# gchq/annchor

Measured on AMD Instinct MI355X. Metric: knn_graph_builds_per_s (1 / Annchor.fit() wall-clock; BASELINE: k-NN graph build time + recall@k), higher is better.
Workload: dtype int32 bit-vectors (Levenshtein) + f64 (bounds/regression/selection); 1 GPU; load_strings Levenshtein N=1600 n_anchors=15 k=25 p_work=0.12 niters=2; parallelism=one GPU

## Files before the change

### annchor_amd/_native.py

```python
import ctypes
import os

import numpy as np

_HERE = os.path.dirname(os.path.abspath(__file__))
LIB_PATH = os.environ.get("ANNCHOR_HIP_LIB", os.path.join(_HERE, "libannchor_hip.so"))

F_D, F_A, F_SID, F_IJS, F_I_PTR, F_I_IDX, F_FEATURES, F_NCM, F_RA, F_LABELS, F_THRESH, F_PROB, F_CAND, F_NEXT, F_DAD = range(1, 16)
_FIELD_DTYPE = {
    F_D: np.float64, F_A: np.int64, F_SID: np.uint64, F_IJS: np.int64, F_I_PTR: np.int64, F_I_IDX: np.int64,
    F_FEATURES: np.float64, F_NCM: np.uint8, F_RA: np.float64, F_LABELS: np.int64, F_THRESH: np.float64,
    F_PROB: np.float64, F_CAND: np.int64, F_NEXT: np.int64, F_DAD: np.float64,
}

METRIC_LEVENSHTEIN, METRIC_EUCLIDEAN_F32, METRIC_EUCLIDEAN_F64, METRIC_WASSERSTEIN = 1, 2, 3, 4
METRIC_COSINE_F32, METRIC_COSINE_F64 = 5, 6
METRIC_DTW_F32, METRIC_DTW_F64 = 7, 8
METRIC_FRECHET_F32, METRIC_FRECHET_F64 = 9, 10

_vp, _i32, _i64, _dbl = ctypes.c_void_p, ctypes.c_int32, ctypes.c_int64, ctypes.c_double
_SIGNATURES = {
    "annchor_create": (ctypes.c_int, [ctypes.c_int, ctypes.POINTER(_vp)]),
    "annchor_destroy": (None, [_vp]),
    "annchor_release_parked": (ctypes.c_int, []),
    "annchor_parked_bytes": (ctypes.c_int, [ctypes.c_int, ctypes.POINTER(_i64)]),
    "annchor_last_error": (ctypes.c_char_p, [_vp]),
    "annchor_create_error": (ctypes.c_char_p, []),
    "annchor_device_name": (ctypes.c_int, [_vp, ctypes.c_char_p, ctypes.c_int]),
    "annchor_device_pci_bus_id": (ctypes.c_int, [ctypes.c_int, ctypes.c_char_p, ctypes.c_int]),
    "annchor_device_mem_info": (ctypes.c_int, [ctypes.c_int, ctypes.POINTER(_i64), ctypes.POINTER(_i64)]),
    "annchor_synchronize": (ctypes.c_int, [_vp]),
    "annchor_lev_persist_state": (ctypes.c_int, [ctypes.c_int]),
    "annchor_last_kernel_ms": (ctypes.c_int, [_vp, ctypes.POINTER(ctypes.c_float)]),
    "annchor_set_strings": (ctypes.c_int, [_vp, _vp, _vp, _vp, _i64, _i32]),
    "annchor_set_strings_u16": (ctypes.c_int, [_vp, _vp, _vp, _vp, _i64, _i32]),
    "annchor_set_points_f32": (ctypes.c_int, [_vp, _vp, _i64, _i32]),
    "annchor_set_points_f64": (ctypes.c_int, [_vp, _vp, _i64, _i32]),
    "annchor_set_points_cosine_f32": (ctypes.c_int, [_vp, _vp, _i64, _i32]),
    "annchor_set_points_cosine_f64": (ctypes.c_int, [_vp, _vp, _i64, _i32]),
    "annchor_set_series_f32": (ctypes.c_int, [_vp, _vp, _vp, _vp, _i64, _i32]),
    "annchor_set_series_f64": (ctypes.c_int, [_vp, _vp, _vp, _vp, _i64, _i32]),
    "annchor_set_curves_f32": (ctypes.c_int, [_vp, _vp, _vp, _vp, _i64, _i32]),
    "annchor_set_curves_f64": (ctypes.c_int, [_vp, _vp, _vp, _vp, _i64, _i32]),
    "annchor_set_histograms": (ctypes.c_int, [_vp, _vp, _i64, _i32, _vp]),
    "annchor_set_histograms_wide": (ctypes.c_int, [_vp, _vp, _i64, _i32, _vp]),
    "annchor_set_opaque": (ctypes.c_int, [_vp, _i64]),
    "annchor_metric_pairs": (ctypes.c_int, [_vp, _vp, _i64, _vp]),
# ... 351 lines not shown
        except Exception:
            pass

    def _chk(self, rc):
        if rc != 0:
            raise NativeError("libannchor_hip error %d: %s" % (rc, self.lib.annchor_last_error(self.h).decode()))

    def device_name(self):
        buf = ctypes.create_string_buffer(256)
        self._chk(self.lib.annchor_device_name(self.h, buf, 256))
        return buf.value.decode()

    def synchronize(self):
        self._chk(self.lib.annchor_synchronize(self.h))

    def last_kernel_ms(self):
        ms = ctypes.c_float()
        self._chk(self.lib.annchor_last_kernel_ms(self.h, ctypes.byref(ms)))
        return ms.value

    def set_strings(self, codes, offs, lens, alphabet):
        offs, lens = _c(offs, np.int64), _c(lens, np.int32)
        if np.asarray(codes).dtype == np.uint16:
            codes = _c(codes, np.uint16)
            self._chk(self.lib.annchor_set_strings_u16(self.h, _ptr(codes), _ptr(offs), _ptr(lens), len(lens), int(alphabet)))
        else:
            codes = _c(codes, np.uint8)
            self._chk(self.lib.annchor_set_strings(self.h, _ptr(codes), _ptr(offs), _ptr(lens), len(lens), int(alphabet)))
        self.nx, self.metric = len(lens), METRIC_LEVENSHTEIN

# ... 677 lines not shown
```

### annchor_amd/csrc/common.h

```cpp
#pragma once
#include <hip/hip_runtime.h>

#include <cstdint>
#include <cstdio>
#include <cstring>
#include <string>
#include <vector>
#include <chrono>

#include "../../include/annchor_hip.h"

#define ANN_WAVE 64

struct DevBuf {
    void *p = nullptr;
    size_t cap = 0;
    bool in_arena = false;
    template <typename T> T *as() const { return reinterpret_cast<T *>(p); }
};

struct ProfEntry {
    const char *name;
    double ms = 0;
    int64_t launches = 0;
// ... 15 lines not shown
    size_t arena_size = 0, arena_off = 0;

    int metric = ANNCHOR_METRIC_NONE;
    int64_t nx = 0;
    DevBuf sym, soff, slen;
    int alphabet = 0, maxlen = 0;
    bool sym_wide = false;
    int lev_gl0 = 0;
    double lev_frac0 = 0.0;
    DevBuf lev_order;
    int lev_nshort = 0;
    DevBuf lev_ap;
    DevBuf lev_ap_min;
    uint32_t lev_ap_epoch = 0;
    uint32_t lev_ap_probe_epoch = 0;
    DevBuf lev_cursors;
    int lev_cursor_epoch = 0;
    DevBuf lev_perm;
    DevBuf pts;
    int dtw_window = -1;
    int curve_dim = 0;
    int dim = 0;
    DevBuf hist, cost, supp;
    DevBuf hs_bin, hs_val, hs_cnt;
    int nbins = 0, max_support = 0;
    double cost_max = 0.0;
    int emd_epoch = 0;
    bool cost_is_metric = false;
    bool hist_integral = false;
    bool hist_fits_i16 = false;
// ... 121 lines not shown
        int _r = (expr);             \
        if (_r != ANNCHOR_OK) return _r; \
    } while (0)

#define ANN_REQUIRE(c, cond, code, ...)    \
    do {                                   \
        if (!(cond)) {                     \
            ann_set_err((c), __VA_ARGS__); \
            return (code);                 \
        }                                  \
    } while (0)

int ann_reserve(annchor_ctx *c, DevBuf &b, size_t bytes);
int ann_arena_init(annchor_ctx *c, int64_t nx);
int ann_prewarm_state(annchor_ctx *c);
void ann_lev_ap_probe(annchor_ctx *c);
size_t ann_sel2_table_bytes();
size_t ann_tie_hist_bytes();
size_t ann_sel_state_bytes();
int ann_h2d(annchor_ctx *c, void *dst, const void *src, size_t bytes);
hipError_t ann_sync(annchor_ctx *c, const char *where);
int ann_dev_alloc(annchor_ctx *c, void **p, size_t want, size_t *got);
void ann_dev_free(annchor_ctx *c, void *p, size_t bytes);
struct Sel2Epilogue;
int ann_kth_async(annchor_ctx *c, const double *vals, const uint8_t *flag, int64_t n, const int64_t *ks, int nk,
                  const unsigned long long **d_prefix, const int **d_unfinished, const Sel2Epilogue *epi = nullptr);
void ann_kth_async_done(annchor_ctx *c);
int ann_d2h(annchor_ctx *c, void *dst, const void *src, size_t bytes);
int ann_d2h_then(annchor_ctx *c, void *dst, const void *src, size_t bytes, int (*then)(annchor_ctx *));
int ann_d2h2(annchor_ctx *c, void *dst1, const void *src1, size_t bytes1, void *dst2, const void *src2, size_t bytes2);
// ... 169 lines not shown
```

### annchor_amd/csrc/ctx.hip

```cpp
#include <cstdarg>
#include <cmath>
#include <cstdlib>

#include "common.h"
#include <algorithm>
#include <chrono>
#include <mutex>

static std::string g_create_err;
void ann_stream_release(annchor_ctx *c);
void ann_enemies_release(annchor_ctx *c);
void ann_comm_release(annchor_ctx *c);
hipError_t ann_comm_guarded_sync(annchor_ctx *c, hipStream_t stream, const char *where);

const char *ann_set_err(annchor_ctx *c, const char *fmt, ...)
{
    char buf[1024];
    va_list ap;
    va_start(ap, fmt);
    vsnprintf(buf, sizeof buf, fmt, ap);
    va_end(ap);
    if (c && c->comm_aborted && c->err.rfind("collective timed out", 0) == 0) return c->err.c_str();
    if (c) c->err = buf; else g_create_err = buf;
    return c ? c->err.c_str() : g_create_err.c_str();
// ... 608 lines not shown
    }
    ANN_TRY(ann_arena_init(c, nx));
    ANN_TRY(ann_prewarm_state(c));
    ANN_TRY(ann_reserve(c, c->sym, pool.size() * sizeof(uint16_t)));
    ANN_TRY(ann_reserve(c, c->soff, sizeof(int32_t) * (size_t)nx));
    ANN_TRY(ann_reserve(c, c->slen, sizeof(int32_t) * (size_t)nx));
    ANN_TRY(ann_h2d(c, c->sym.p, pool.data(), pool.size() * sizeof(uint16_t)));
    ANN_TRY(ann_h2d(c, c->soff.p, o.data(), sizeof(int32_t) * (size_t)nx));
    ANN_TRY(ann_h2d(c, c->slen.p, lens, sizeof(int32_t) * (size_t)nx));
    c->metric = ANNCHOR_METRIC_LEVENSHTEIN;
    c->nx = nx;
    c->alphabet = alphabet;
    c->maxlen = maxlen;
    c->sym_wide = true;
    c->lev_gl0 = 0; c->lev_frac0 = 0.0; c->lev_nshort = 0;
    reset_pipeline(c);
    return ANNCHOR_OK;
}

extern "C" int annchor_set_strings(annchor_ctx *c, const uint8_t *symbols, const int64_t *offs,
                                   const int32_t *lens, int64_t nx, int32_t alphabet)
{
    if (!c || !symbols || !offs || !lens) return ANNCHOR_EINVAL;
    ANN_REQUIRE(c, nx > 1 && nx < (1ll << 31), ANNCHOR_ELIMIT, "nx=%lld out of range", (long long)nx);
    ANN_REQUIRE(c, alphabet >= 1 && alphabet <= 256, ANNCHOR_ELIMIT, "alphabet=%d not in 1..256", alphabet);
    ANN_CHECK_HIP(c, hipSetDevice(c->device));
    std::vector<int32_t> o((size_t)nx);
    size_t total = 0;
    int maxlen = 0;
    for (int64_t s = 0; s < nx; ++s) {
// ... 22 lines not shown
    c->metric = ANNCHOR_METRIC_LEVENSHTEIN;
    c->nx = nx;
    c->alphabet = alphabet;
    c->maxlen = maxlen;
    c->sym_wide = false;
    {
        std::vector<int32_t> ord((size_t)nx);
        int64_t ns = 0;
        for (int64_t s = 0; s < nx; ++s) ns += lens[s] <= 512;
        int64_t a = 0, b = ns;
        for (int64_t s = 0; s < nx; ++s) ord[(size_t)(lens[s] <= 512 ? a++ : b++)] = (int32_t)s;
        ANN_TRY(ann_reserve(c, c->lev_order, sizeof(int32_t) * (size_t)nx));
        ANN_TRY(ann_h2d(c, c->lev_order.p, ord.data(), sizeof(int32_t) * (size_t)nx));
        c->lev_nshort = (int)ns;
    }
    {
        const int W = (maxlen + 31) / 32 > 0 ? (maxlen + 31) / 32 : 1;
        c->lev_gl0 = 0;
        c->lev_frac0 = 0.0;
        if (W <= 32) {
            const int gl0 = 64 / (64 / W + 1);
            if (gl0 >= 1) {
                int64_t cnt = 0;
                for (int64_t s = 0; s < nx; ++s) cnt += (lens[s] + 31) / 32 <= gl0;
                c->lev_gl0 = gl0;
                c->lev_frac0 = (double)cnt / (double)nx;
            }
        }
    }
    reset_pipeline(c);
// ... 295 lines not shown
```

### annchor_amd/csrc/lev.hip

```cpp
#include <cstdlib>

#include "common.h"
#include <atomic>
#include <type_traits>

#define LEV_THREADS 256
#define LEV_WAVES (LEV_THREADS / ANN_WAVE)

__device__ __forceinline__ uint32_t dpp_wave_shr1(uint32_t v)
{
    return (uint32_t)__builtin_amdgcn_update_dpp((int)v, (int)v, 0x138 , 0xf, 0xf, false);
}

struct LevArgs {
    const uint8_t *sym;
    const int32_t *soff;
    const int32_t *slen;
    const int2 *ij;
    const int32_t *idx;
    const int32_t *anchor;
    int64_t n;
    double *out;
    double *RA;
    uint8_t *ncm;
// ... 899 lines not shown
    }
}


struct LevArgsAP {
    const uint8_t *sym;
    const int32_t *soff;
    const int32_t *slen;
    const int32_t *order;
    double *Dt;
    int32_t *A;
    int32_t *rank;
    unsigned long long *slots;
    uint32_t *abort_epoch;
    uint16_t *rescue_min;
    long long timeout_ticks;
    long long *dbg;
    uint32_t epoch;
    int n_short, nx, na, first, ntasks, slot_stride;
    int alphabet, pm_bytes, fb_stride, buf_stride, pad, wave_bytes;
};

template <bool RESCUE> __global__ __launch_bounds__(RESCUE ? 512 : ANN_WAVE) void k_lev_ap(LevArgsAP a)
{
    extern __shared__ __attribute__((aligned(16))) unsigned char smem_all[];
    __shared__ uint32_t s_best;
    __shared__ int32_t s_A[64];
    {
        const uint32_t ab = __hip_atomic_load(a.abort_epoch, __ATOMIC_RELAXED, __HIP_MEMORY_SCOPE_AGENT);
        if (RESCUE ? ab != a.epoch : ab == a.epoch) return;
    }
    const int lane = threadIdx.x & 63, wv = threadIdx.x >> 6, nwv = blockDim.x >> 6;
    unsigned char *smem = smem_all + (size_t)wv * a.wave_bytes;
    const int A = a.alphabet, nx = a.nx;
    unsigned char *pm_col = smem + (size_t)(lane >> 5) * A * LEVF_ROW + (size_t)(lane & 31) * 4;
// ... 6 lines not shown
    uint32_t rm0 = 0xffffu, rm1 = 0xffffu;
    int rk0 = -1, rk1 = -1;
    int si = a.first;
    for (int r = 0; r < a.na; ++r) {
        if (RESCUE) {
            if (threadIdx.x == 0) { s_best = 0; s_A[r] = si; }
            __syncthreads();
        }
#ifdef LEV_AP_PROFILE
#define AP_STAMP(i) do { if (!RESCUE && lane == 0) a.dbg[((size_t)blockIdx.x * 64 + r) * 8 + (i)] = (long long)__builtin_readcyclecounter(); } while (0)
#else
#define AP_STAMP(i) do { } while (0)
#endif
        AP_STAMP(0);
        if ((RESCUE ? threadIdx.x : blockIdx.x + lane) == 0) a.A[r] = si;
        const int la = a.slen[si];
        const uint8_t *asrc = a.sym + a.soff[si];
        uint32_t mykey = 0;
        for (int vb = RESCUE ? wv : (int)blockIdx.x; vb < a.ntasks; vb += RESCUE ? nwv : a.ntasks) {
            if (RESCUE || r == 0) {
                const bool packed = vb < ws;
                const int GL = packed ? 16 : 32;
                const int slot = lane / GL;
                w = lane - slot * GL; pair = slot >> 1; half = slot & 1; LP = packed ? 32 : 64;
                hp_or = w == 0 ? 0x80000000u : 0u;
                hn_and = w == 0 ? 0u : 0xffffffffu;
                asm volatile("" : "+v"(hp_or), "+v"(hn_and));
                tq0 = tq1 = -1;
                if (packed) {
                    tq0 = a.order[2 * vb];
                    if (2 * vb + 1 < a.n_short) tq1 = a.order[2 * vb + 1];
                } else {
                    tq0 = a.order[a.n_short + (vb - ws)];
                }
                for (int e = lane * 16; e < 3 * a.buf_stride; e += 64 * 16) *reinterpret_cast<uint4 *>(bufs + e) = make_uint4(0, 0, 0, 0);
                int ln0 = 0, ln1 = 0;
                {
                    ln0 = a.slen[tq0];
                    const uint8_t *src = a.sym + a.soff[tq0];
                    for (int ch = lane; ch < ((ln0 + 15) >> 4); ch += 64)
                        reinterpret_cast<uint4 *>(bufs + a.pad)[ch] = reinterpret_cast<const uint4 *>(src)[ch];
                }
                if (tq1 >= 0) {
                    ln1 = a.slen[tq1];
                    const uint8_t *src = a.sym + a.soff[tq1];
                    for (int ch = lane; ch < ((ln1 + 15) >> 4); ch += 64)
                        reinterpret_cast<uint4 *>(bufs + a.buf_stride + a.pad)[ch] = reinterpret_cast<const uint4 *>(src)[ch];
                }
                wave_lds_fence();
                have = pair == 0 || (packed && pair == 1 && tq1 >= 0);
                mytq = !have ? -1 : (pair == 0 ? tq0 : tq1);
                m = !have ? 0 : (pair == 0 ? ln0 : ln1);
                Wp = (m + 31) >> 5;
                const uint8_t *pat = bufs + pair * a.buf_stride + a.pad;
                for (int c = 0; c < A; ++c) *reinterpret_cast<uint32_t *>(pm_col + (size_t)c * LEVF_ROW) = 0u;
                if (have && w < Wp) {
                    const int valid = min(32, m - w * 32);
                    uint32_t sy[32];
                    if (half == 0) {
                        const uint4 *p16 = reinterpret_cast<const uint4 *>(pat + w * 32);
                        const uint4 q0 = p16[0], q1 = p16[1];
                        const uint32_t wd[8] = {q0.x, q0.y, q0.z, q0.w, q1.x, q1.y, q1.z, q1.w};
#pragma unroll
                        for (int k = 0; k < 32; ++k) sy[k] = (wd[k >> 2] >> ((k & 3) * 8)) & 0xffu;
                    } else {
#pragma unroll
                        for (int k = 0; k < 32; ++k) sy[k] = pat[max(m - 1 - (w * 32 + k), 0)];
                    }
#pragma unroll
                    for (int k = 0; k < 32; ++k)
                        if (k < valid) atomicOr(reinterpret_cast<uint32_t *>(pm_col + (size_t)sy[k] * LEVF_ROW), 1u << k);
                }
                rows = !have ? 0u : (w < Wp - 1 ? 0xffffffffu : (w == Wp - 1 ? (0xffffffffu >> (31 - ((m - 1) & 31))) : 0u));
            }
            for (int ch = lane; ch < ((la + 15) >> 4); ch += 64)
                reinterpret_cast<uint4 *>(bufs + 2 * a.buf_stride + a.pad)[ch] = reinterpret_cast<const uint4 *>(asrc)[ch];
            wave_lds_fence();
            AP_STAMP(1);
            const uint8_t *txt = bufs + 2 * a.buf_stride + a.pad;
            const int n = have ? la : 0;
            const int h = (n + 1) >> 1;
            const uint32_t un = (have && m > 0) ? (uint32_t)(half ? n - h : h) : 0u;
            int max_steps = (have && m > 0) ? h + Wp - 1 : 0;
            int k_lo = (have && m > 0) ? Wp - 1 : 0, k_hi = (have && m > 0) ? n - h : 0x7fffffff;
#pragma unroll
            for (int off = 32; off > 0; off >>= 1) {
                max_steps = max(max_steps, __shfl_xor(max_steps, off));
                k_lo = max(k_lo, __shfl_xor(k_lo, off));
                k_hi = min(k_hi, __shfl_xor(k_hi, off));
            }
            max_steps = __builtin_amdgcn_readfirstlane(max_steps);
// ... 51 lines not shown
            for (; k < k_hi; ++k) column1(k, std::false_type());
            for (; k < max_steps; ++k) column1(k, std::true_type());
            AP_STAMP(3);

            const int part = __popc(vp & rows) - __popc(vn & rows);
            int incl = part;
#pragma unroll
            for (int off = 1; off < 32; off <<= 1) {
                const int o = __shfl_up(incl, off, 32);
                if (w >= off) incl += o;
            }
            int val = (int)un + incl - part;
            if (m == 0) val = half ? n - h : h;
            int16_t *fbp = FB + (size_t)pair * 2 * a.fb_stride;
            int16_t *fb = fbp + (size_t)half * a.fb_stride;
            if (have && w == 0) fb[0] = (int16_t)val;
#pragma unroll
            for (int b = 0; b < 32; ++b) {
                val += (int)((vp >> b) & 1u) - (int)((vn >> b) & 1u);
                if ((rows >> b) & 1u) fb[w * 32 + b + 1] = (int16_t)val;
            }
            wave_lds_fence();
            int best = 0x7fffffff;
            const int lp = lane & (LP - 1);
            if (have)
                for (int i = lp; i <= m; i += LP) best = min(best, (int)fbp[i] + (int)fbp[a.fb_stride + m - i]);
#pragma unroll
            for (int off = 32; off > 0; off >>= 1)
                if (off < LP) best = min(best, __shfl_xor(best, off));
            if (have && lp == 0) a.Dt[(size_t)r * nx + mytq] = (double)best;
            wave_lds_fence();
            AP_STAMP(4);
            if (RESCUE) {
                if (have && lp == 0) {
                    uint32_t v = (uint32_t)best;
                    if (r > 1) v = min(v, (uint32_t)a.rescue_min[mytq]);
                    a.rescue_min[mytq] = (uint16_t)v;
                    atomicMax(&s_best, (v << 16) | (uint32_t)(0xffff - mytq));
                }
            } else {
                const uint32_t d0 = (uint32_t)__shfl(best, 0), d1 = (uint32_t)__shfl(best, 32);
                rm0 = r <= 1 ? d0 : min(rm0, d0);
                rm1 = r <= 1 ? d1 : min(rm1, d1);
                mykey = (rm0 << 16) | (uint32_t)(0xffff - tq0);
                if (tq1 >= 0) mykey = max(mykey, (rm1 << 16) | (uint32_t)(0xffff - tq1));
                if (si == tq0) rk0 = r;
                if (si == tq1) rk1 = r;
            }
        }
        if (r + 1 == a.na) break;
        if (RESCUE) {
            __syncthreads();
            si = 0xffff - (int)(s_best & 0xffffu);
            __syncthreads();
        } else {
            const uint32_t tag = a.epoch * 64u + (uint32_t)r;
            unsigned long long *sl = a.slots + (size_t)(r & 1) * a.slot_stride;
            unsigned long long *pl = sl + 2 * a.slot_stride;
            const int ngroups = (a.ntasks + 63) >> 6;
            if (lane == 0)
                __hip_atomic_store(sl + blockIdx.x, ((unsigned long long)tag << 32) | mykey, __ATOMIC_RELAXED, __HIP_MEMORY_SCOPE_AGENT);
            const long long t0 = wall_clock64();
            AP_STAMP(5);
            uint32_t mx;
            bool collected = (int)blockIdx.x >= ngroups;
            int polls = 0;
            for (;;) {
                if (!collected) {
                    const unsigned long long v = __hip_atomic_load(sl + min((int)blockIdx.x * 64 + lane, a.ntasks - 1), __ATOMIC_RELAXED,
                                                                   __HIP_MEMORY_SCOPE_AGENT);
                    if (__all((uint32_t)(v >> 32) == tag)) {
                        uint32_t gm = (uint32_t)v;
#pragma unroll
                        for (int off = 32; off > 0; off >>= 1) gm = max(gm, (uint32_t)__shfl_xor((int)gm, off));
                        if (lane == 0)
                            __hip_atomic_store(pl + blockIdx.x, ((unsigned long long)tag << 32) | gm, __ATOMIC_RELAXED, __HIP_MEMORY_SCOPE_AGENT);
// ... 19 lines not shown
            AP_STAMP(6);
        }
    }
    if (RESCUE) {
        __syncthreads();
        for (int j = threadIdx.x; j < nx; j += blockDim.x) a.rank[j] = -1;
        __syncthreads();
        if (threadIdx.x == 0)
            for (int r = 0; r < a.na; ++r) a.rank[s_A[r]] = r;
    } else {
        if (lane == 0) {
            a.rank[tq0] = rk0;
            if (tq1 >= 0) a.rank[tq1] = rk1;
        }
    }
}

static int launch_p2(annchor_ctx *c, const PairSource &src, double *d_out, double *d_RA, uint8_t *d_ncm)
{
    LevArgsP2 a;
    a.sym = c->sym.as<uint8_t>(); a.soff = c->soff.as<int32_t>(); a.slen = c->slen.as<int32_t>();
    a.ij = src.ij; a.idx = src.idx; a.n = src.n; a.out = d_out; a.RA = d_RA; a.ncm = d_ncm;
    a.alphabet = c->alphabet;
    a.pm_bytes = 2 * a.alphabet * LEVF_ROW;
    a.fb_stride = (c->maxlen + 2 + 7) & ~7;
    a.pad = ((c->maxlen / 2 + 48) + 15) & ~15;
    a.buf_stride = 2 * a.pad + ((c->maxlen + 15) & ~15) + 16;
    const size_t lds = (size_t)a.pm_bytes + 4 * (size_t)a.buf_stride + 4 * sizeof(int16_t) * a.fb_stride;
    ANN_REQUIRE(c, lds <= 160 * 1024, ANNCHOR_ELIMIT, "alphabet %d x length %d needs %zu B of LDS (> 160 KiB)", c->alphabet,
                c->maxlen, lds);
// ... 72 lines not shown
    if (set == 1) { g_lev_ap_off.store(0); g_lev_ap_strikes.store(0); }
    return g_lev_ap_off.load() ? 0 : 1;
}

int ann_lev_anchor_rounds(annchor_ctx *c, int32_t na, int32_t first, bool *done)
{
    *done = false;
    {
        const char *e = getenv("ANNCHOR_LEV_PERSIST");
        if (e && atoi(e) == 0) return ANNCHOR_OK;
        if (g_lev_ap_off.load()) return ANNCHOR_OK;
        const char *e_a = getenv("ANNCHOR_LEV_ANCHOR"), *e_r = getenv("ANNCHOR_LEV_R");
        if ((e_a && atoi(e_a) != 2) || e_r) return ANNCHOR_OK;
    }
    if (c->metric != ANNCHOR_METRIC_LEVENSHTEIN || c->sym_wide || !c->lev_order.p) return ANNCHOR_OK;
    if ((c->maxlen + 31) / 32 > 32 || c->nx > 8192 || na < 1 || na > 64) return ANNCHOR_OK;
    LevArgsAP a;
    a.ntasks = (c->lev_nshort + 1) / 2 + (int)(c->nx - c->lev_nshort);
    if (a.ntasks > 1024) return ANNCHOR_OK;
    a.alphabet = c->alphabet;
    a.pm_bytes = 2 * a.alphabet * LEVF_ROW;
    a.fb_stride = (c->maxlen + 2 + 7) & ~7;
    a.pad = ((c->maxlen / 2 + 48) + 15) & ~15;
    a.buf_stride = 2 * a.pad + ((c->maxlen + 15) & ~15) + 16;
    a.wave_bytes = (int)(((size_t)a.pm_bytes + 3 * (size_t)a.buf_stride + 4 * sizeof(int16_t) * a.fb_stride + 15) & ~(size_t)15);
    size_t lds = (size_t)a.wave_bytes;
    if (lds > 160 * 1024) return ANNCHOR_OK;
    if (a.ntasks <= c->prop.multiProcessorCount * 4 && lds < (size_t)40 * 1024) lds = (size_t)40 * 1024;
    if (lds > 64 * 1024)
        ANN_CHECK_HIP(c, hipFuncSetAttribute((const void *)k_lev_ap<false>, hipFuncAttributeMaxDynamicSharedMemorySize, (int)lds));
    int per_cu = 0;
    ANN_CHECK_HIP(c, hipOccupancyMaxActiveBlocksPerMultiprocessor(&per_cu, k_lev_ap<false>, ANN_WAVE, lds));
    if ((int64_t)per_cu * c->prop.multiProcessorCount < a.ntasks) return ANNCHOR_OK;
    int rwaves = (int)std::min<size_t>(8, (160 * 1024 - 1024) / (size_t)a.wave_bytes);
// ... 4 lines not shown
    a.slot_stride = 1024;
    const size_t slot_bytes = sizeof(unsigned long long) * 4 * (size_t)a.slot_stride;
    if (!c->lev_ap.p) {
        ANN_TRY(ann_reserve(c, c->lev_ap, slot_bytes + 64));
        ANN_CHECK_HIP(c, hipMemsetAsync(c->lev_ap.p, 0, slot_bytes + 64, c->stream));
        c->lev_ap_epoch = 0;
    }
    ANN_TRY(ann_reserve(c, c->lev_ap_min, sizeof(uint16_t) * (size_t)c->nx));
    ANN_TRY(ann_reserve(c, c->anchorRank, sizeof(int32_t) * (size_t)c->nx));
    a.sym = c->sym.as<uint8_t>(); a.soff = c->soff.as<int32_t>(); a.slen = c->slen.as<int32_t>();
    a.order = c->lev_order.as<int32_t>();
    a.Dt = c->Dt.as<double>(); a.A = c->A.as<int32_t>(); a.rank = c->anchorRank.as<int32_t>();
    a.slots = c->lev_ap.as<unsigned long long>();
    a.abort_epoch = reinterpret_cast<uint32_t *>(c->lev_ap.as<unsigned char>() + slot_bytes);
    a.rescue_min = c->lev_ap_min.as<uint16_t>();
    {
        const char *e = getenv("ANNCHOR_LEV_PERSIST_TIMEOUT_US");
        a.timeout_ticks = (e ? atoll(e) : 20000ll) * 100;
    }
    a.dbg = nullptr;
#ifdef LEV_AP_PROFILE
    {
        static long long *dbg = nullptr;
        if (!dbg) (void)hipMalloc(&dbg, sizeof(long long) * 1024 * 64 * 8);
        a.dbg = dbg;
    }
#endif
    a.epoch = ++c->lev_ap_epoch;
    if ((a.epoch & 0x3ffffffu) == 0) a.epoch = c->lev_ap_epoch = 1;
    a.n_short = c->lev_nshort; a.nx = (int)c->nx; a.na = na; a.first = first;
// ... 4 lines not shown
        k_lev_ap<true><<<1, rwaves * ANN_WAVE, rlds, c->stream>>>(a);
    }
    if (c->pin) {
        unsigned char *tail = c->pin + (size_t)annchor_ctx::PIN_SLOTS * annchor_ctx::PIN_SLOT_BYTES + annchor_ctx::PIN_DL_BYTES;
        ANN_CHECK_HIP(c, hipMemcpyAsync(tail, a.abort_epoch, 4, hipMemcpyDeviceToHost, c->stream));
        c->lev_ap_probe_epoch = a.epoch;
    }
    ANN_CHECK_HIP(c, hipGetLastError());
#ifdef LEV_AP_PROFILE
    {
        static int calls = 0;
        if (++calls == 5) {
            std::vector<long long> h((size_t)1024 * 64 * 8);
            (void)hipStreamSynchronize(c->stream);
            (void)hipMemcpy(h.data(), a.dbg, h.size() * sizeof(long long), hipMemcpyDeviceToHost);
            const char *nm[6] = {"stage anchor", "loop setup", "columns", "prefix+combine", "key", "barrier"};
            for (int b : {0, 1, 500, 700, a.ntasks - 1}) {
                fprintf(stderr, "k_lev_ap wave %d:", b);
                for (int ph = 0; ph < 6; ++ph) {
                    double sum = 0;
                    for (int r = 0; r + 1 < na; ++r) sum += (double)(h[((size_t)b * 64 + r) * 8 + ph + 1] - h[((size_t)b * 64 + r) * 8 + ph]);
                    fprintf(stderr, " %s %.0f", nm[ph], sum / (na - 1));
                }
                fprintf(stderr, " | round %.0f (s_memtime ticks per round)\n", (double)(h[((size_t)b * 64 + na - 2) * 8 + 6] - h[(size_t)b * 64 * 8]) / (na - 1));
            }
        }
    }
#endif
    *done = true;
    return ANNCHOR_OK;
}

struct LevArgsW {
    const uint16_t *sym;
    const int32_t *soff;
    const int32_t *slen;
    const int2 *ij;
    const int32_t *idx;
    const int32_t *anchor;
    int64_t n;
// ... 187 lines not shown
```

### include/annchor_hip.h

```cpp
#ifndef ANNCHOR_HIP_H
#define ANNCHOR_HIP_H

#include <stdint.h>

#ifdef __cplusplus
extern "C" {
#endif

typedef struct annchor_ctx annchor_ctx;

enum {
    ANNCHOR_OK = 0,
    ANNCHOR_EINVAL = -1,
    ANNCHOR_EHIP = -2,
    ANNCHOR_ENODEV = -3,
    ANNCHOR_ELIMIT = -4,
    ANNCHOR_ESTATE = -5
};

enum { ANNCHOR_METRIC_NONE = 0, ANNCHOR_METRIC_LEVENSHTEIN = 1, ANNCHOR_METRIC_EUCLIDEAN_F32 = 2,
       ANNCHOR_METRIC_EUCLIDEAN_F64 = 3, ANNCHOR_METRIC_WASSERSTEIN = 4, ANNCHOR_METRIC_COSINE_F32 = 5,
       ANNCHOR_METRIC_COSINE_F64 = 6, ANNCHOR_METRIC_DTW_F32 = 7, ANNCHOR_METRIC_DTW_F64 = 8,
       ANNCHOR_METRIC_FRECHET_F32 = 9, ANNCHOR_METRIC_FRECHET_F64 = 10 };

// ... 106 lines not shown
int annchor_download_samples(annchor_ctx *ctx, int64_t *positions, double *feats, double *sample_y, double *sample_predict);
int annchor_fit_regression_device(annchor_ctx *ctx, const double *bins, int32_t nbins, int32_t first_iteration, int32_t is_metric);
int annchor_fit_errors_device(annchor_ctx *ctx);
int annchor_model_download(annchor_ctx *ctx, double *W, double *c, int32_t *status, int64_t *err_ptr, int32_t *flags );
int annchor_errors_download(annchor_ctx *ctx, double *errs, int64_t n_errs);
int annchor_model_download_with_errors(annchor_ctx *ctx, double *W, double *c, int32_t *status, int64_t *err_ptr, int32_t *flags ,
                                       double *errs, int64_t errs_cap, int64_t *n_errs);

int annchor_select_candidates(annchor_ctx *ctx, int32_t n_neighbors, int32_t nmin, const double *errs,
                              const int64_t *err_ptr, int32_t nlabels, int64_t n_refine,
                              int32_t lookahead, int64_t *n_cand, int64_t *n_next);
int annchor_select_prepare(annchor_ctx *ctx, int32_t n_neighbors, int32_t nmin);
int annchor_mark_candidates(annchor_ctx *ctx);
int annchor_refine_candidates(annchor_ctx *ctx);
int annchor_lev_persist_state(int set);

int annchor_park_refine(annchor_ctx *ctx, int32_t action);
int annchor_set_refined(annchor_ctx *ctx, const double *exact, int64_t n_cand);

int annchor_update_bounds(annchor_ctx *ctx);

int annchor_neighbor_graph(annchor_ctx *ctx, int32_t n_neighbors, int64_t *ng_idx, double *ng_dist);

int annchor_stream_bind(annchor_ctx *ctx, const float *X, int64_t n_local, int32_t dim, int64_t global_base,
                        int32_t x_on_device);
int annchor_stream_anchor_round(annchor_ctx *ctx, const float *anchor_vec, int32_t round, int32_t n_anchors,
                                double *local_max, int64_t *local_arg);
int annchor_stream_get_row(annchor_ctx *ctx, int64_t local_idx, float *out);
int annchor_stream_order(annchor_ctx *ctx, int32_t min_tiles, void **Xs, void **rs, void **perm, void **lo, void **hi,
                         void **mid, int64_t *n_pad, int32_t *n_tiles, int32_t *dim_padded);
// ... 102 lines not shown
```

Before: 360.7 graphs/s.

## Precompute Levenshtein pattern match masks and padded string pool at bind time

At set_strings time, two new kernels build a padded per-string byte pool and per-task bit-parallel match-mask tables. The persistent anchor-pick kernel then copies these precomputed masks into LDS instead of staging pattern strings and building masks with LDS atomics every round, and keeps the anchor text in registers. It also vectorizes the forward/backward prefix stores and the min-combine scan using popcount and uint4 accesses. The per-round slot publish is moved earlier, before the Dt write. This adds bind-time work and up to 32 MB of device memory, and exposes a debug accessor for the tables.

```diff
diff --git a/annchor_amd/_native.py b/annchor_amd/_native.py
--- a/annchor_amd/_native.py
+++ b/annchor_amd/_native.py
@@ -31,6 +31,7 @@
     "annchor_device_mem_info": (ctypes.c_int, [ctypes.c_int, ctypes.POINTER(_i64), ctypes.POINTER(_i64)]),
     "annchor_synchronize": (ctypes.c_int, [_vp]),
     "annchor_lev_persist_state": (ctypes.c_int, [ctypes.c_int]),
+    "annchor_lev_bound_tables": (ctypes.c_int, [_vp, _i32, _vp, _i64]),
     "annchor_last_kernel_ms": (ctypes.c_int, [_vp, ctypes.POINTER(ctypes.c_float)]),
     "annchor_set_strings": (ctypes.c_int, [_vp, _vp, _vp, _vp, _i64, _i32]),
     "annchor_set_strings_u16": (ctypes.c_int, [_vp, _vp, _vp, _vp, _i64, _i32]),
@@ -412,6 +413,18 @@
     def synchronize(self):
         self._chk(self.lib.annchor_synchronize(self.h))
 
+    def lev_bound_tables(self):
+        info = np.zeros(4, dtype=np.int32)
+        self._chk(self.lib.annchor_lev_bound_tables(self.h, 0, _ptr(info), info.nbytes))
+        tasks, alphabet, stride, kept = (int(v) for v in info)
+        pool = np.zeros((self.nx, stride), dtype=np.uint8)
+        self._chk(self.lib.annchor_lev_bound_tables(self.h, 2, _ptr(pool), pool.nbytes))
+        masks = None
+        if kept:
+            masks = np.zeros((tasks, 2, alphabet, 32), dtype=np.uint32)
+            self._chk(self.lib.annchor_lev_bound_tables(self.h, 1, _ptr(masks), masks.nbytes))
+        return pool, masks
+
     def last_kernel_ms(self):
         ms = ctypes.c_float()
         self._chk(self.lib.annchor_last_kernel_ms(self.h, ctypes.byref(ms)))
diff --git a/annchor_amd/csrc/common.h b/annchor_amd/csrc/common.h
--- a/annchor_amd/csrc/common.h
+++ b/annchor_amd/csrc/common.h
@@ -53,6 +53,10 @@
     DevBuf lev_ap_min;
     uint32_t lev_ap_epoch = 0;
     uint32_t lev_ap_probe_epoch = 0;
+    DevBuf lev_pool;
+    int lev_pool_stride = 0;
+    DevBuf lev_masks;
+    int lev_masks_tasks = 0;
     DevBuf lev_cursors;
     int lev_cursor_epoch = 0;
     DevBuf lev_perm;
@@ -204,6 +208,7 @@
 int ann_reserve(annchor_ctx *c, DevBuf &b, size_t bytes);
 int ann_arena_init(annchor_ctx *c, int64_t nx);
 int ann_prewarm_state(annchor_ctx *c);
+int ann_lev_bind_tables(annchor_ctx *c);
 void ann_lev_ap_probe(annchor_ctx *c);
 size_t ann_sel2_table_bytes();
 size_t ann_tie_hist_bytes();
diff --git a/annchor_amd/csrc/ctx.hip b/annchor_amd/csrc/ctx.hip
--- a/annchor_amd/csrc/ctx.hip
+++ b/annchor_amd/csrc/ctx.hip
@@ -646,6 +646,7 @@
     c->maxlen = maxlen;
     c->sym_wide = true;
     c->lev_gl0 = 0; c->lev_frac0 = 0.0; c->lev_nshort = 0;
+    c->lev_pool_stride = 0; c->lev_masks_tasks = 0;
     reset_pipeline(c);
     return ANNCHOR_OK;
 }
@@ -698,6 +699,7 @@
         ANN_TRY(ann_h2d(c, c->lev_order.p, ord.data(), sizeof(int32_t) * (size_t)nx));
         c->lev_nshort = (int)ns;
     }
+    ANN_TRY(ann_lev_bind_tables(c));
     {
         const int W = (maxlen + 31) / 32 > 0 ? (maxlen + 31) / 32 : 1;
         c->lev_gl0 = 0;
diff --git a/annchor_amd/csrc/lev.hip b/annchor_amd/csrc/lev.hip
--- a/annchor_amd/csrc/lev.hip
+++ b/annchor_amd/csrc/lev.hip
@@ -937,11 +937,13 @@
     unsigned long long *slots;
     uint32_t *abort_epoch;
     uint16_t *rescue_min;
+    const uint8_t *pool;
+    const uint32_t *masks;
     long long timeout_ticks;
     long long *dbg;
     uint32_t epoch;
     int n_short, nx, na, first, ntasks, slot_stride;
-    int alphabet, pm_bytes, fb_stride, buf_stride, pad, wave_bytes;
+    int alphabet, pm_bytes, fb_stride, buf_stride, pad, wave_bytes, pool_stride;
 };
 
 template <bool RESCUE> __global__ __launch_bounds__(RESCUE ? 512 : ANN_WAVE) void k_lev_ap(LevArgsAP a)
@@ -978,8 +980,9 @@
 #endif
         AP_STAMP(0);
         if ((RESCUE ? threadIdx.x : blockIdx.x + lane) == 0) a.A[r] = si;
+        uint4 atext = make_uint4(0, 0, 0, 0);
+        if (lane * 16 < a.pool_stride) atext = *reinterpret_cast<const uint4 *>(a.pool + (size_t)si * a.pool_stride + lane * 16);
         const int la = a.slen[si];
-        const uint8_t *asrc = a.sym + a.soff[si];
         uint32_t mykey = 0;
         for (int vb = RESCUE ? wv : (int)blockIdx.x; vb < a.ntasks; vb += RESCUE ? nwv : a.ntasks) {
             if (RESCUE || r == 0) {
@@ -997,48 +1000,52 @@
                 } else {
                     tq0 = a.order[a.n_short + (vb - ws)];
                 }
-                for (int e = lane * 16; e < 3 * a.buf_stride; e += 64 * 16) *reinterpret_cast<uint4 *>(bufs + e) = make_uint4(0, 0, 0, 0);
-                int ln0 = 0, ln1 = 0;
-                {
-                    ln0 = a.slen[tq0];
-                    const uint8_t *src = a.sym + a.soff[tq0];
-                    for (int ch = lane; ch < ((ln0 + 15) >> 4); ch += 64)
-                        reinterpret_cast<uint4 *>(bufs + a.pad)[ch] = reinterpret_cast<const uint4 *>(src)[ch];
-                }
-                if (tq1 >= 0) {
-                    ln1 = a.slen[tq1];
-                    const uint8_t *src = a.sym + a.soff[tq1];
-                    for (int ch = lane; ch < ((ln1 + 15) >> 4); ch += 64)
-                        reinterpret_cast<uint4 *>(bufs + a.buf_stride + a.pad)[ch] = reinterpret_cast<const uint4 *>(src)[ch];
-                }
-                wave_lds_fence();
+                const int ln0 = a.slen[tq0], ln1 = tq1 >= 0 ? a.slen[tq1] : 0;
                 have = pair == 0 || (packed && pair == 1 && tq1 >= 0);
                 mytq = !have ? -1 : (pair == 0 ? tq0 : tq1);
                 m = !have ? 0 : (pair == 0 ? ln0 : ln1);
                 Wp = (m + 31) >> 5;
-                const uint8_t *pat = bufs + pair * a.buf_stride + a.pad;
-                for (int c = 0; c < A; ++c) *reinterpret_cast<uint32_t *>(pm_col + (size_t)c * LEVF_ROW) = 0u;
-                if (have && w < Wp) {
-                    const int valid = min(32, m - w * 32);
-                    uint32_t sy[32];
-                    if (half == 0) {
-                        const uint4 *p16 = reinterpret_cast<const uint4 *>(pat + w * 32);
-                        const uint4 q0 = p16[0], q1 = p16[1];
-                        const uint32_t wd[8] = {q0.x, q0.y, q0.z, q0.w, q1.x, q1.y, q1.z, q1.w};
-#pragma unroll
-                        for (int k = 0; k < 32; ++k) sy[k] = (wd[k >> 2] >> ((k & 3) * 8)) & 0xffu;
-                    } else {
-#pragma unroll
-                        for (int k = 0; k < 32; ++k) sy[k] = pat[max(m - 1 - (w * 32 + k), 0)];
+                if (a.masks) {
+                    const uint4 *src = reinterpret_cast<const uint4 *>(a.masks + (size_t)vb * (a.pm_bytes >> 2));
+                    for (int e = lane; e < (a.pm_bytes >> 4); e += 64) reinterpret_cast<uint4 *>(smem)[e] = src[e];
+                    for (int e = lane * 16; e < a.buf_stride; e += 64 * 16)
+                        *reinterpret_cast<uint4 *>(bufs + 2 * a.buf_stride + e) = make_uint4(0, 0, 0, 0);
+                } else {
+                    for (int e = lane * 16; e < 3 * a.buf_stride; e += 64 * 16) *reinterpret_cast<uint4 *>(bufs + e) = make_uint4(0, 0, 0, 0);
+                    {
+                        const uint8_t *src = a.sym + a.soff[tq0];
+                        for (int ch = lane; ch < ((ln0 + 15) >> 4); ch += 64)
+                            reinterpret_cast<uint4 *>(bufs + a.pad)[ch] = reinterpret_cast<const uint4 *>(src)[ch];
                     }
-#pragma unroll
-                    for (int k = 0; k < 32; ++k)
-                        if (k < valid) atomicOr(reinterpret_cast<uint32_t *>(pm_col + (size_t)sy[k] * LEVF_ROW), 1u << k);
+                    if (tq1 >= 0) {
+                        const uint8_t *src = a.sym + a.soff[tq1];
+                        for (int ch = lane; ch < ((ln1 + 15) >> 4); ch += 64)
+                            reinterpret_cast<uint4 *>(bufs + a.buf_stride + a.pad)[ch] = reinterpret_cast<const uint4 *>(src)[ch];
+                    }
+                    wave_lds_fence();
+                    const uint8_t *pat = bufs + pair * a.buf_stride + a.pad;
+                    for (int c = 0; c < A; ++c) *reinterpret_cast<uint32_t *>(pm_col + (size_t)c * LEVF_ROW) = 0u;
+                    if (have && w < Wp) {
+                        const int valid = min(32, m - w * 32);
+                        uint32_t sy[32];
+                        if (half == 0) {
+                            const uint4 *p16 = reinterpret_cast<const uint4 *>(pat + w * 32);
+                            const uint4 q0 = p16[0], q1 = p16[1];
+                            const uint32_t wd[8] = {q0.x, q0.y, q0.z, q0.w, q1.x, q1.y, q1.z, q1.w};
+#pragma unroll
+                            for (int k = 0; k < 32; ++k) sy[k] = (wd[k >> 2] >> ((k & 3) * 8)) & 0xffu;
+                        } else {
+#pragma unroll
+                            for (int k = 0; k < 32; ++k) sy[k] = pat[max(m - 1 - (w * 32 + k), 0)];
+                        }
+#pragma unroll
+                        for (int k = 0; k < 32; ++k)
+                            if (k < valid) atomicOr(reinterpret_cast<uint32_t *>(pm_col + (size_t)sy[k] * LEVF_ROW), 1u << k);
+                    }
                 }
                 rows = !have ? 0u : (w < Wp - 1 ? 0xffffffffu : (w == Wp - 1 ? (0xffffffffu >> (31 - ((m - 1) & 31))) : 0u));
             }
-            for (int ch = lane; ch < ((la + 15) >> 4); ch += 64)
-                reinterpret_cast<uint4 *>(bufs + 2 * a.buf_stride + a.pad)[ch] = reinterpret_cast<const uint4 *>(asrc)[ch];
+            if (lane * 16 < a.pool_stride) *reinterpret_cast<uint4 *>(bufs + 2 * a.buf_stride + a.pad + lane * 16) = atext;
             wave_lds_fence();
             AP_STAMP(1);
             const uint8_t *txt = bufs + 2 * a.buf_stride + a.pad;
@@ -1120,23 +1127,44 @@
             if (m == 0) val = half ? n - h : h;
             int16_t *fbp = FB + (size_t)pair * 2 * a.fb_stride;
             int16_t *fb = fbp + (size_t)half * a.fb_stride;
-            if (have && w == 0) fb[0] = (int16_t)val;
-#pragma unroll
-            for (int b = 0; b < 32; ++b) {
-                val += (int)((vp >> b) & 1u) - (int)((vn >> b) & 1u);
-                if ((rows >> b) & 1u) fb[w * 32 + b + 1] = (int16_t)val;
+            {
+                const uint32_t vpr = vp & rows, vnr = vn & rows;
+                uint32_t q[16];
+#pragma unroll
+                for (int j = 0; j < 32; j += 2) {
+                    const uint32_t m0 = j ? (0xffffffffu >> (32 - j)) : 0u, m1 = 0xffffffffu >> (31 - j);
+                    const int lo = val + __popc(vpr & m0) - __popc(vnr & m0);
+                    const int hi = val + __popc(vpr & m1) - __popc(vnr & m1);
+                    q[j >> 1] = ((uint32_t)lo & 0xffffu) | ((uint32_t)hi << 16);
+                }
+                if (have && w * 32 <= m) {
+                    uint4 *dst = reinterpret_cast<uint4 *>(fb + w * 32);
+#pragma unroll
+                    for (int e = 0; e < 4; ++e)
+                        if (w * 32 + e * 8 <= m) dst[e] = make_uint4(q[4 * e], q[4 * e + 1], q[4 * e + 2], q[4 * e + 3]);
+                }
+                if (have && m > 0 && w == Wp - 1 && (m & 31) == 0) fb[m] = (int16_t)(val + __popc(vpr) - __popc(vnr));
             }
             wave_lds_fence();
             int best = 0x7fffffff;
             const int lp = lane & (LP - 1);
-            if (have)
-                for (int i = lp; i <= m; i += LP) best = min(best, (int)fbp[i] + (int)fbp[a.fb_stride + m - i]);
+            if (have) {
+                const int16_t *bq = fbp + a.fb_stride + m;
+                for (int i = lp * 8; i <= m; i += LP * 8) {
+                    const uint4 fv = *reinterpret_cast<const uint4 *>(fbp + i);
+                    const uint32_t fw[4] = {fv.x, fv.y, fv.z, fv.w};
+                    int16_t bw[8];
+                    __builtin_memcpy(bw, bq - i - 7, 16);
+#pragma unroll
+                    for (int e = 0; e < 8; ++e) {
+                        const int f = (int)(int16_t)(fw[e >> 1] >> ((e & 1) * 16));
+                        if (i + e <= m) best = min(best, f + (int)bw[7 - e]);
+                    }
+                }
+            }
 #pragma unroll
             for (int off = 32; off > 0; off >>= 1)
                 if (off < LP) best = min(best, __shfl_xor(best, off));
-            if (have && lp == 0) a.Dt[(size_t)r * nx + mytq] = (double)best;
-            wave_lds_fence();
-            AP_STAMP(4);
             if (RESCUE) {
                 if (have && lp == 0) {
                     uint32_t v = (uint32_t)best;
@@ -1152,7 +1180,14 @@
                 if (tq1 >= 0) mykey = max(mykey, (rm1 << 16) | (uint32_t)(0xffff - tq1));
                 if (si == tq0) rk0 = r;
                 if (si == tq1) rk1 = r;
-            }
+                if (r + 1 < a.na && lane == 0)
+                    __hip_atomic_store(a.slots + (size_t)(r & 1) * a.slot_stride + blockIdx.x,
+                                       ((unsigned long long)(a.epoch * 64u + (uint32_t)r) << 32) | mykey, __ATOMIC_RELAXED,
+                                       __HIP_MEMORY_SCOPE_AGENT);
+            }
+            AP_STAMP(4);
+            if (have && lp == 0) a.Dt[(size_t)r * nx + mytq] = (double)best;
+            wave_lds_fence();
         }
         if (r + 1 == a.na) break;
         if (RESCUE) {
@@ -1164,8 +1199,6 @@
             unsigned long long *sl = a.slots + (size_t)(r & 1) * a.slot_stride;
             unsigned long long *pl = sl + 2 * a.slot_stride;
             const int ngroups = (a.ntasks + 63) >> 6;
-            if (lane == 0)
-                __hip_atomic_store(sl + blockIdx.x, ((unsigned long long)tag << 32) | mykey, __ATOMIC_RELAXED, __HIP_MEMORY_SCOPE_AGENT);
             const long long t0 = wall_clock64();
             AP_STAMP(5);
             uint32_t mx;
@@ -1215,6 +1248,103 @@
             if (tq1 >= 0) a.rank[tq1] = rk1;
         }
     }
+}
+
+__global__ __launch_bounds__(ANN_WAVE) void k_lev_bind_pool(const uint8_t *__restrict__ sym, const int32_t *__restrict__ soff,
+                                                            const int32_t *__restrict__ slen, uint8_t *__restrict__ pool, int stride)
+{
+    const int s = blockIdx.x, lane = threadIdx.x;
+    const int chunks = (slen[s] + 15) >> 4;
+    const uint4 *src = reinterpret_cast<const uint4 *>(sym + soff[s]);
+    for (int ch = lane; ch * 16 < stride; ch += ANN_WAVE)
+        reinterpret_cast<uint4 *>(pool + (size_t)s * stride)[ch] = ch < chunks ? src[ch] : make_uint4(0, 0, 0, 0);
+}
+
+__global__ __launch_bounds__(ANN_WAVE) void k_lev_bind_masks(const uint8_t *__restrict__ pool, const int32_t *__restrict__ slen,
+                                                             const int32_t *__restrict__ order, uint32_t *__restrict__ masks,
+                                                             int stride, int n_short, int alphabet)
+{
+    const int vb = blockIdx.x, lane = threadIdx.x;
+    const int ws = (n_short + 1) >> 1;
+    const bool packed = vb < ws;
+    const int GL = packed ? 16 : 32;
+    const int slot = lane / GL, w = lane - slot * GL, pair = slot >> 1, half = slot & 1;
+    int tq = -1;
+    if (packed) {
+        if (2 * vb + pair < n_short) tq = order[2 * vb + pair];
+    } else if (pair == 0) {
+        tq = order[n_short + (vb - ws)];
+    }
+    const int m = tq >= 0 ? slen[tq] : 0;
+    const int valid = min(32, m - w * 32);
+    uint32_t sy[32];
+#pragma unroll
+    for (int k = 0; k < 32; ++k) {
+        const int pos = half ? m - 1 - (w * 32 + k) : w * 32 + k;
+        sy[k] = k < valid ? (uint32_t)pool[(size_t)tq * stride + pos] : 0xffffffffu;
+    }
+    uint32_t *row = masks + ((size_t)vb * 2 + (lane >> 5)) * alphabet * 32 + (lane & 31);
+    for (int c = 0; c < alphabet; ++c) {
+        uint32_t word = 0;
+#pragma unroll
+        for (int k = 0; k < 32; ++k) word |= (sy[k] == (uint32_t)c ? 1u : 0u) << k;
+        row[(size_t)c * 32] = word;
+    }
+}
+
+static bool lev_ap_shape_ok(const annchor_ctx *c, int *ntasks)
+{
+    *ntasks = (c->lev_nshort + 1) / 2 + (int)(c->nx - c->lev_nshort);
+    return !c->sym_wide && (c->maxlen + 31) / 32 <= 32 && c->nx <= 8192 && *ntasks <= 1024;
+}
+
+static const size_t LEV_BOUND_MASKS_CAP = (size_t)32 << 20;
+
+int ann_lev_bind_tables(annchor_ctx *c)
+{
+    c->lev_pool_stride = 0;
+    c->lev_masks_tasks = 0;
+    int ntasks = 0;
+    if (!lev_ap_shape_ok(c, &ntasks)) return ANNCHOR_OK;
+    const int stride = std::max(16, (c->maxlen + 15) & ~15);
+    ANN_TRY(ann_reserve(c, c->lev_pool, (size_t)c->nx * stride));
+    k_lev_bind_pool<<<(int)c->nx, ANN_WAVE, 0, c->stream>>>(c->sym.as<uint8_t>(), c->soff.as<int32_t>(), c->slen.as<int32_t>(),
+                                                            c->lev_pool.as<uint8_t>(), stride);
+    ANN_CHECK_HIP(c, hipGetLastError());
+    c->lev_pool_stride = stride;
+    const size_t mask_bytes = (size_t)ntasks * 2 * c->alphabet * LEVF_ROW;
+    if (mask_bytes > LEV_BOUND_MASKS_CAP) return ANNCHOR_OK;
+    ANN_TRY(ann_reserve(c, c->lev_masks, mask_bytes));
+    k_lev_bind_masks<<<ntasks, ANN_WAVE, 0, c->stream>>>(c->lev_pool.as<uint8_t>(), c->slen.as<int32_t>(), c->lev_order.as<int32_t>(),
+                                                         c->lev_masks.as<uint32_t>(), stride, c->lev_nshort, c->alphabet);
+    ANN_CHECK_HIP(c, hipGetLastError());
+    c->lev_masks_tasks = ntasks;
+    return ANNCHOR_OK;
+}
+
+extern "C" int annchor_lev_bound_tables(annchor_ctx *c, int32_t what, void *dst, int64_t n_bytes)
+{
+    if (!c || !dst) return ANNCHOR_EINVAL;
+    ANN_REQUIRE(c, c->metric == ANNCHOR_METRIC_LEVENSHTEIN && c->lev_pool_stride > 0, ANNCHOR_EINVAL,
+                "no bound Levenshtein tables (byte strings of <= 1024 symbols, <= 8192 of them)");
+    int ntasks = 0;
+    lev_ap_shape_ok(c, &ntasks);
+    if (what == 0) {
+        ANN_REQUIRE(c, n_bytes == 16, ANNCHOR_EINVAL, "info is int32 [4]");
+        const int32_t info[4] = {ntasks, c->alphabet, c->lev_pool_stride, c->lev_masks_tasks > 0 ? 1 : 0};
+        memcpy(dst, info, 16);
+        return ANNCHOR_OK;
+    }
+    if (what == 1) {
+        ANN_REQUIRE(c, c->lev_masks_tasks > 0, ANNCHOR_EINVAL, "the match-mask tables of this set are above the cap");
+        const size_t bytes = (size_t)ntasks * 2 * c->alphabet * LEVF_ROW;
+        ANN_REQUIRE(c, n_bytes == (int64_t)bytes, ANNCHOR_EINVAL, "the tables have %zu bytes", bytes);
+        return ann_d2h(c, dst, c->lev_masks.p, bytes);
+    }
+    ANN_REQUIRE(c, what == 2, ANNCHOR_EINVAL, "what=%d not in 0..2", what);
+    const size_t bytes = (size_t)c->nx * c->lev_pool_stride;
+    ANN_REQUIRE(c, n_bytes == (int64_t)bytes, ANNCHOR_EINVAL, "the strings have %zu bytes", bytes);
+    return ann_d2h(c, dst, c->lev_pool.p, bytes);
 }
 
 static int launch_p2(annchor_ctx *c, const PairSource &src, double *d_out, double *d_RA, uint8_t *d_ncm)
@@ -1317,10 +1447,8 @@
         if ((e_a && atoi(e_a) != 2) || e_r) return ANNCHOR_OK;
     }
     if (c->metric != ANNCHOR_METRIC_LEVENSHTEIN || c->sym_wide || !c->lev_order.p) return ANNCHOR_OK;
-    if ((c->maxlen + 31) / 32 > 32 || c->nx > 8192 || na < 1 || na > 64) return ANNCHOR_OK;
     LevArgsAP a;
-    a.ntasks = (c->lev_nshort + 1) / 2 + (int)(c->nx - c->lev_nshort);
-    if (a.ntasks > 1024) return ANNCHOR_OK;
+    if (!lev_ap_shape_ok(c, &a.ntasks) || c->lev_pool_stride <= 0 || na < 1 || na > 64) return ANNCHOR_OK;
     a.alphabet = c->alphabet;
     a.pm_bytes = 2 * a.alphabet * LEVF_ROW;
     a.fb_stride = (c->maxlen + 2 + 7) & ~7;
@@ -1355,6 +1483,12 @@
     a.slots = c->lev_ap.as<unsigned long long>();
     a.abort_epoch = reinterpret_cast<uint32_t *>(c->lev_ap.as<unsigned char>() + slot_bytes);
     a.rescue_min = c->lev_ap_min.as<uint16_t>();
+    a.pool = c->lev_pool.as<uint8_t>(); a.pool_stride = c->lev_pool_stride;
+    a.masks = c->lev_masks_tasks == a.ntasks ? c->lev_masks.as<uint32_t>() : nullptr;
+    {
+        const char *e = getenv("ANNCHOR_LEV_BOUND_MASKS");
+        if (e && atoi(e) == 0) a.masks = nullptr;
+    }
     {
         const char *e = getenv("ANNCHOR_LEV_PERSIST_TIMEOUT_US");
         a.timeout_ticks = (e ? atoll(e) : 20000ll) * 100;
@@ -1389,16 +1523,20 @@
             std::vector<long long> h((size_t)1024 * 64 * 8);
             (void)hipStreamSynchronize(c->stream);
             (void)hipMemcpy(h.data(), a.dbg, h.size() * sizeof(long long), hipMemcpyDeviceToHost);
-            const char *nm[6] = {"stage anchor", "loop setup", "columns", "prefix+combine", "key", "barrier"};
-            for (int b : {0, 1, 500, 700, a.ntasks - 1}) {
-                fprintf(stderr, "k_lev_ap wave %d:", b);
-                for (int ph = 0; ph < 6; ++ph) {
-                    double sum = 0;
-                    for (int r = 0; r + 1 < na; ++r) sum += (double)(h[((size_t)b * 64 + r) * 8 + ph + 1] - h[((size_t)b * 64 + r) * 8 + ph]);
-                    fprintf(stderr, " %s %.0f", nm[ph], sum / (na - 1));
-                }
-                fprintf(stderr, " | round %.0f (s_memtime ticks per round)\n", (double)(h[((size_t)b * 64 + na - 2) * 8 + 6] - h[(size_t)b * 64 * 8]) / (na - 1));
-            }
+            auto med = [](std::vector<double> &v) { std::sort(v.begin(), v.end()); return v.empty() ? 0.0 : v[v.size() / 2]; };
+            auto phase = [&](int lo, int hi, int r0, int r1) {
+                std::vector<double> v;
+                for (int b = 0; b < a.ntasks; ++b)
+                    for (int r = r0; r < r1; ++r) v.push_back((double)(h[((size_t)b * 64 + r) * 8 + hi] - h[((size_t)b * 64 + r) * 8 + lo]));
+                return med(v);
+            };
+            fprintf(stderr, "k_lev_ap stamps (shader clock ticks, median over %d waves): masks %s\n", a.ntasks, a.masks ? "bound" : "in-kernel");
+            fprintf(stderr, "  round 0     : setup %.0f columns %.0f epilogue %.0f arrive %.0f barrier %.0f\n", phase(0, 2, 0, 1), phase(2, 3, 0, 1),
+                    phase(3, 4, 0, 1), phase(4, 5, 0, 1), phase(5, 6, 0, 1));
+            if (na > 2)
+                fprintf(stderr, "  rounds 1..%-2d: setup %.0f (stage %.0f + loop setup %.0f) columns %.0f epilogue %.0f arrive %.0f barrier %.0f | round %.0f\n",
+                        na - 2, phase(0, 2, 1, na - 1), phase(0, 1, 1, na - 1), phase(1, 2, 1, na - 1), phase(2, 3, 1, na - 1),
+                        phase(3, 4, 1, na - 1), phase(4, 5, 1, na - 1), phase(5, 6, 1, na - 1), phase(0, 6, 1, na - 1));
         }
     }
 #endif
diff --git a/include/annchor_hip.h b/include/annchor_hip.h
--- a/include/annchor_hip.h
+++ b/include/annchor_hip.h
@@ -144,6 +144,7 @@
 int annchor_mark_candidates(annchor_ctx *ctx);
 int annchor_refine_candidates(annchor_ctx *ctx);
 int annchor_lev_persist_state(int set);
+int annchor_lev_bound_tables(annchor_ctx *ctx, int32_t what, void *dst, int64_t n_bytes);
 
 int annchor_park_refine(annchor_ctx *ctx, int32_t action);
 int annchor_set_refined(annchor_ctx *ctx, const double *exact, int64_t n_cand);
```

Result: slower. 354.3 graphs/s (-1.8%).
